# serizard/DeltaKD

Hardware: NVIDIA B200
Metric: distill-loss fwd+bwd samples/s (higher is better)
Workload: dtype bf16

## Files before the change

deltakd_b200/csrc/common.cuh:

```cuda
#pragma once
#include <cuda_bf16.h>
#include <cuda_runtime.h>
#include <stdint.h>
#include <stdio.h>

#include "../../include/deltakd.h"

#if defined(__CUDA_ARCH__) && (__CUDA_ARCH__ < 1000)
#error "libdeltakd_sm100 is written for sm_100a (B200) only"
#endif

namespace dkd {

void set_error(const char* fmt, ...);
int check_launch(const char* what);

#define DKD_REQUIRE(cond, code, ...)  \
  do {                                \
    if (!(cond)) {                    \
      ::dkd::set_error(__VA_ARGS__);  \
      return (code);                  \
    }                                 \
  } while (0)

// ... 164 lines not shown
__device__ __forceinline__ float2 add2(float2 a, float2 b) {
  unsigned long long r;
  asm("add.rn.f32x2 %0, %1, %2;" : "=l"(r) : "l"(f2_pack(a.x, a.y)), "l"(f2_pack(b.x, b.y)));
  return f2_unpack(r);
}
__device__ __forceinline__ float2 sub2(float2 a, float2 b) {
  unsigned long long r;
  asm("sub.rn.f32x2 %0, %1, %2;" : "=l"(r) : "l"(f2_pack(a.x, a.y)), "l"(f2_pack(b.x, b.y)));
  return f2_unpack(r);
}
__device__ __forceinline__ float2 mul2(float2 a, float2 b) {
  unsigned long long r;
  asm("mul.rn.f32x2 %0, %1, %2;" : "=l"(r) : "l"(f2_pack(a.x, a.y)), "l"(f2_pack(b.x, b.y)));
  return f2_unpack(r);
}
__device__ __forceinline__ float2 splat2(float x) { return make_float2(x, x); }

__device__ __forceinline__ float warp_sum(float v) {
#pragma unroll
  for (int o = 16; o > 0; o >>= 1) v += __shfl_xor_sync(0xffffffffu, v, o);
  return v;
}
__device__ __forceinline__ float warp_max(float v) {
#pragma unroll
  for (int o = 16; o > 0; o >>= 1) v = fmaxf(v, __shfl_xor_sync(0xffffffffu, v, o));
  return v;
}
__device__ __forceinline__ double warp_sum(double v) {
#pragma unroll
  for (int o = 16; o > 0; o >>= 1) v += __shfl_xor_sync(0xffffffffu, v, o);
  return v;
}

template <int K, int THREADS>
__device__ __forceinline__ void block_sum(float (&v)[K], float* scratch) {
  constexpr int WARPS = THREADS / 32;
  const int lane = threadIdx.x & 31, warp = threadIdx.x >> 5;
#pragma unroll
  for (int k = 0; k < K; ++k) v[k] = warp_sum(v[k]);
  if constexpr (THREADS == 32) return;
  __syncthreads();
  if (lane == 0) {
#pragma unroll
    for (int k = 0; k < K; ++k) scratch[k * WARPS + warp] = v[k];
  }
  __syncthreads();
#pragma unroll
  for (int k = 0; k < K; ++k) {
    float a = 0.f;
#pragma unroll
    for (int w = 0; w < WARPS; ++w) a += scratch[k * WARPS + w];
    v[k] = a;
  }
}
template <int K, int THREADS>
__device__ __forceinline__ void block_max(float (&v)[K], float* scratch) {
  constexpr int WARPS = THREADS / 32;
  const int lane = threadIdx.x & 31, warp = threadIdx.x >> 5;
#pragma unroll
  for (int k = 0; k < K; ++k) v[k] = warp_max(v[k]);
  if constexpr (THREADS == 32) return;
  __syncthreads();
  if (lane == 0) {
#pragma unroll
    for (int k = 0; k < K; ++k) scratch[k * WARPS + warp] = v[k];
  }
// ... 12 lines not shown
```

deltakd_b200/csrc/logit_kd.cu:

```cuda
#include <stdlib.h>

#include "common.cuh"

#ifndef DKD_LOGIT_STAMP
#define DKD_LOGIT_STAMP(point, dep) ((void)0)
#endif

namespace dkd {
namespace {

constexpr int kThreads = 128;

__device__ __forceinline__ float fexp(float x) {
  float y;
  asm("ex2.approx.ftz.f32 %0, %1;" : "=f"(y) : "f"(x * 1.4426950408889634f));
  return y;
}
__device__ __forceinline__ float fexp2(float x, float k2, float m2) {
  float y;
  asm("ex2.approx.ftz.f32 %0, %1;" : "=f"(y) : "f"(fmaf(x, k2, -m2)));
  return y;
}

__device__ __forceinline__ float2 ex2_2(float2 x) {
  float2 y;
  asm("ex2.approx.ftz.f32 %0, %1;" : "=f"(y.x) : "f"(x.x));
  asm("ex2.approx.ftz.f32 %0, %1;" : "=f"(y.y) : "f"(x.y));
  return y;
}

struct LogitKdParams {
  const void* z;
  const void* zk;
  const void* zt;
  const void* y;
  void* gz;
  void* gzk;
  float* loss_out;
  float* row_base;
  float* row_kd;
  unsigned int* ticket;
  int64_t B, C;
  int label_kind, kd_kind;
  float smoothing, alpha, tau;
  const float* mix_lam;
};

constexpr int kRuntimeMode = -2;
constexpr float kL2e = 1.4426950408889634f;
template <typename T, int VEC, int NV, int THREADS = kThreads, int LK = kRuntimeMode, int KK = kRuntimeMode,
          bool PACK2 = (THREADS == kThreads), typename Publish>
__device__ __forceinline__ void logit_row(const LogitKdParams& p, int64_t row, const T* z, const T* zk, const T* zt, const T* y,
                                          T* gz_row, T* gzk_row, float* scratch, int* s_arg, float* s_argv, float& base_out,
                                          float& kd_out, Publish&& publish) {
  const int64_t C = p.C;
  const int label_kind = LK == kRuntimeMode ? p.label_kind : LK;
  const int kd_kind = KK == kRuntimeMode ? p.kd_kind : KK;
  const int tid = THREADS == 32 ? (int)(threadIdx.x & 31) : (int)threadIdx.x;
  const int64_t label = label_kind == 1 ? reinterpret_cast<const int64_t*>(p.y)[row] : -1;
  const bool mixing = label_kind == 1 && p.mix_lam != nullptr;
  const int64_t label2 = mixing ? reinterpret_cast<const int64_t*>(p.y)[p.B - 1 - row] : -1;
  const float lam = mixing ? __ldg(p.mix_lam) : 1.f;
  const float invT = kd_kind == 1 ? 1.f / p.tau : 1.f;

  constexpr int NVR = NV > 0 ? NV : 1;
  float rz[NVR][VEC], rk[NVR][VEC], rt[NVR][VEC], ry[NVR][VEC];
  const int nchunk = (int)((C + (int64_t)THREADS * VEC - 1) / ((int64_t)THREADS * VEC));

  auto col_of = [&](int it) -> int64_t { return ((int64_t)it * THREADS + tid) * VEC; };
  const T* any = label_kind >= 0 ? z : zk;
  const T* lz = label_kind >= 0 ? z : any;
  const T* lzk = kd_kind ? zk : any;
  const T* lzt = kd_kind ? zt : any;
  const T* ly = label_kind == 0 ? y : any;
  auto load4 = [&](int it, float (&a)[VEC], float (&b)[VEC], float (&c)[VEC], float (&d)[VEC]) {
    const int64_t col0 = col_of(it);
    const int64_t col = col0 < C ? col0 : 0;
    Vec<T, VEC>::load(lz + col, a);
    Vec<T, VEC>::load(lzk + col, b);
    Vec<T, VEC>::load(lzt + col, c);
    Vec<T, VEC>::load(ly + col, d);
    if (label_kind < 0) {
#pragma unroll
      for (int v = 0; v < VEC; ++v) a[v] = 0.f;
    }
  };

  float mx[3] = {-INFINITY, -INFINITY, -INFINITY};
  float best = -INFINITY;
  int64_t best_i = INT64_MAX;
  auto pass1 = [&](int it, float (&a)[VEC], float (&b)[VEC], float (&c)[VEC]) {
    const int64_t col = col_of(it);
    if (col < C) {
#pragma unroll
      for (int v = 0; v < VEC; ++v) {
        mx[0] = fmaxf(mx[0], a[v]);
        if (kd_kind) {
          mx[1] = fmaxf(mx[1], b[v]);
          mx[2] = fmaxf(mx[2], c[v]);
          if (kd_kind == 2 && c[v] > best) { best = c[v]; best_i = col + v; }
        }
      }
    }
  };
  if constexpr (NV > 0) {
#pragma unroll
    for (int it = 0; it < NV; ++it)
      if (it < nchunk) load4(it, rz[it], rk[it], rt[it], ry[it]);
#pragma unroll
    for (int it = 0; it < NV; ++it)
      if (it < nchunk) pass1(it, rz[it], rk[it], rt[it]);
  } else {
    for (int it = 0; it < nchunk; ++it) {
      load4(it, rz[0], rk[0], rt[0], ry[0]);
      pass1(it, rz[0], rk[0], rt[0]);
    }
  }
  DKD_LOGIT_STAMP(1, mx[0]);
  block_max<3, THREADS>(mx, scratch);
  DKD_LOGIT_STAMP(2, mx[0]);
  mx[1] *= invT;
  mx[2] *= invT;
  int64_t tgt = label;
  int64_t hard_idx = -1;
  if (kd_kind == 2) {
    float bv = best;
    long long bi = (long long)best_i;
#pragma unroll
    for (int o = 16; o > 0; o >>= 1) {
      float ov = __shfl_xor_sync(0xffffffffu, bv, o);
      long long oi = __shfl_xor_sync(0xffffffffu, bi, o);
      if (ov > bv || (ov == bv && oi < bi)) { bv = ov; bi = oi; }
    }
    if constexpr (THREADS > 32) {
      __syncthreads();
      if ((threadIdx.x & 31) == 0) { s_argv[threadIdx.x >> 5] = bv; s_arg[threadIdx.x >> 5] = (int)bi; }
      __syncthreads();
      bv = s_argv[0]; bi = s_arg[0];
#pragma unroll
      for (int w = 1; w < THREADS / 32; ++w) {
        if (s_argv[w] > bv || (s_argv[w] == bv && s_arg[w] < bi)) { bv = s_argv[w]; bi = s_arg[w]; }
      }
    }
    hard_idx = bi;
  }
  (void)tgt;

  float st8[8] = {0.f, 0.f, 0.f, 0.f, 0.f, 0.f, 0.f, 0.f};
  float (&s)[4] = *reinterpret_cast<float(*)[4]>(&st8[0]);
  float (&t)[4] = *reinterpret_cast<float(*)[4]>(&st8[4]);
  constexpr bool PACKED = NV > 0 && VEC % 2 == 0 && PACK2;
  float2 S2[4], T2[2];
#pragma unroll
  for (int k = 0; k < 4; ++k) S2[k] = make_float2(0.f, 0.f);
  T2[0] = T2[1] = make_float2(0.f, 0.f);
  auto pass2 = [&](int it, float (&a)[VEC], float (&b)[VEC], float (&c)[VEC], float (&d)[VEC]) {
    const int64_t col = col_of(it);
    if (col < C) {
      if constexpr (PACKED) {
        const float2 kz = splat2(kL2e), nm0 = splat2(-mx[0] * kL2e);
        const float2 kt = splat2(invT * kL2e), nm1 = splat2(-mx[1] * kL2e), nm2 = splat2(-mx[2] * kL2e);
#pragma unroll
        for (int v = 0; v < VEC; v += 2) {
          const float2 A = make_float2(a[v], a[v + 1]);
          const float2 ea = ex2_2(fma2(A, kz, nm0));
          S2[0] = add2(S2[0], ea);
          if (label_kind == 0) {
            const float2 D = make_float2(d[v], d[v + 1]);
            T2[0] = add2(T2[0], D);
            T2[1] = fma2(D, A, T2[1]);
          } else {
            T2[1] = add2(T2[1], A);
            if (col + v == label) t[2] = a[v];
            if (col + v + 1 == label) t[2] = a[v + 1];
            if (col + v == label2) t[0] = a[v];
            if (col + v + 1 == label2) t[0] = a[v + 1];
          }
          a[v] = ea.x; a[v + 1] = ea.y;
          if (kd_kind == 1) {
            const float2 Bv = make_float2(b[v], b[v + 1]), Cv = make_float2(c[v], c[v + 1]);
            const float2 eb = ex2_2(fma2(Cv, kt, nm2)), es = ex2_2(fma2(Bv, kt, nm1));
            S2[1] = add2(S2[1], es);
            S2[2] = add2(S2[2], eb);
            S2[3] = fma2(eb, sub2(Cv, Bv), S2[3]);
            b[v] = es.x; b[v + 1] = es.y;
            c[v] = eb.x; c[v + 1] = eb.y;
          } else if (kd_kind == 2) {
            const float2 Bv = make_float2(b[v], b[v + 1]);
            const float2 es = ex2_2(fma2(Bv, kz, nm1));
            S2[1] = add2(S2[1], es);
            if (col + v == hard_idx) t[3] = b[v];
            if (col + v + 1 == hard_idx) t[3] = b[v + 1];
            b[v] = es.x; b[v + 1] = es.y;
          }
        }
        return;
      }
#pragma unroll
      for (int v = 0; v < VEC; ++v) {
        const float ea = fexp2(a[v], kL2e, mx[0] * kL2e);
        s[0] += ea;
        if (label_kind == 0) { t[0] += d[v]; t[1] += d[v] * a[v]; }
        else { t[1] += a[v]; if (col + v == label) t[2] = a[v]; if (col + v == label2) t[0] = a[v]; }
        if (NV > 0) a[v] = ea;
        if (kd_kind == 1) {
          const float eb = fexp2(c[v], invT * kL2e, mx[2] * kL2e), es = fexp2(b[v], invT * kL2e, mx[1] * kL2e);
          s[1] += es;
          s[2] += eb;
          s[3] = fmaf(eb, c[v] - b[v], s[3]);
          if (NV > 0) { b[v] = es; c[v] = eb; }
        } else if (kd_kind == 2) {
          const float es = fexp2(b[v], kL2e, mx[1] * kL2e);
          s[1] += es;
          if (col + v == hard_idx) t[3] = b[v];
          if (NV > 0) b[v] = es;
        }
      }
    }
  };
  if constexpr (NV > 0) {
#pragma unroll
    for (int it = 0; it < NV; ++it) if (it < nchunk) pass2(it, rz[it], rk[it], rt[it], ry[it]);
  } else {
    for (int it = 0; it < nchunk; ++it) {
      load4(it, rz[0], rk[0], rt[0], ry[0]);
      pass2(it, rz[0], rk[0], rt[0], ry[0]);
    }
  }
  if constexpr (PACKED) {
#pragma unroll
    for (int k = 0; k < 4; ++k) s[k] = S2[k].x + S2[k].y;
    if (label_kind == 0) t[0] = T2[0].x + T2[0].y;
    t[1] = T2[1].x + T2[1].y;
  }
  block_sum<8, THREADS>(st8, scratch);
  DKD_LOGIT_STAMP(3, s[0]);
  s[3] *= invT;

  const float Bf = (float)p.B, Cf = (float)C;
  const float lse0 = mx[0] + __logf(s[0]);
  float base_row, kd_row = 0.f;
  if (label_kind < 0) base_row = 0.f;
  else if (label_kind == 0) base_row = lse0 * t[0] - t[1];
  else base_row = (1.f - p.smoothing) * (lse0 - (lam * t[2] + (1.f - lam) * t[0])) + p.smoothing * (lse0 - t[1] / Cf);
  float lse1 = 0.f, lse2 = 0.f;
  if (kd_kind == 1) {
    lse1 = mx[1] + __logf(s[1]);
    lse2 = mx[2] + __logf(s[2]);
    kd_row = __fdividef(s[3], s[2]) - lse2 + lse1;
  } else if (kd_kind == 2) {
    lse1 = mx[1] + __logf(s[1]);
    kd_row = lse1 - t[3];
  }
  publish(base_row, kd_row);

  const float wb = (kd_kind == 0 ? 1.f : 1.f - p.alpha) / Bf;
  const float wk = kd_kind == 1 ? p.alpha * p.tau / (Bf * Cf) : p.alpha / Bf;
  const float inv_s0 = __frcp_rn(s[0]), inv_s1 = kd_kind ? __frcp_rn(s[1]) : 0.f, inv_s2 = kd_kind == 1 ? __frcp_rn(s[2]) : 0.f;
  const float k0 = (label_kind == 0 ? inv_s0 * t[0] : inv_s0) * wb;
  const float k1 = inv_s1 * wk, k2 = inv_s2 * wk;
  const float sm_wb = p.smoothing / Cf * wb, hot_wb = (1.f - p.smoothing) * wb * lam, hot2_wb = (1.f - p.smoothing) * wb * (1.f - lam);
  T* gz = label_kind >= 0 ? gz_row : nullptr;
  T* gzk = kd_kind ? gzk_row : nullptr;
  auto pass3 = [&](int it, float (&a)[VEC], float (&b)[VEC], float (&c)[VEC], float (&d)[VEC]) {
    const int64_t col = col_of(it);
    if (col < C) {
      float g0[VEC], g1[VEC];
      if constexpr (PACKED) {
        const float2 K0 = splat2(k0), K1 = splat2(k1), NK2 = splat2(-k2), NWB = splat2(-wb), NSM = splat2(-sm_wb);
#pragma unroll
        for (int v = 0; v < VEC; v += 2) {
          const float2 e0 = make_float2(a[v], a[v + 1]);
          float2 r0;
          if (label_kind == 0) r0 = fma2(e0, K0, mul2(make_float2(d[v], d[v + 1]), NWB));
          else {
            r0 = fma2(e0, K0, NSM);
            if (col + v == label) r0.x -= hot_wb;
            if (col + v + 1 == label) r0.y -= hot_wb;
            if (col + v == label2) r0.x -= hot2_wb;
            if (col + v + 1 == label2) r0.y -= hot2_wb;
          }
          g0[v] = r0.x; g0[v + 1] = r0.y;
          if (kd_kind == 1) {
            const float2 r1 = fma2(make_float2(b[v], b[v + 1]), K1, mul2(make_float2(c[v], c[v + 1]), NK2));
            g1[v] = r1.x; g1[v + 1] = r1.y;
          } else if (kd_kind == 2) {
            float2 r1 = mul2(make_float2(b[v], b[v + 1]), K1);
            if (col + v == hard_idx) r1.x -= wk;
            if (col + v + 1 == hard_idx) r1.y -= wk;
            g1[v] = r1.x; g1[v + 1] = r1.y;
          }
        }
      } else {
// ... 3 lines not shown
        if (label_kind == 0) g0[v] = fmaf(e0, k0, -(d[v] * wb));
        else g0[v] = fmaf(e0, k0, -sm_wb) - (col + v == label ? hot_wb : 0.f) - (col + v == label2 ? hot2_wb : 0.f);
        if (kd_kind == 1) {
          const float es = NV > 0 ? b[v] : fexp(b[v] * invT - mx[1]);
          const float et = NV > 0 ? c[v] : fexp(c[v] * invT - mx[2]);
          g1[v] = fmaf(es, k1, -(et * k2));
        } else if (kd_kind == 2) {
          const float es = NV > 0 ? b[v] : fexp(b[v] - mx[1]);
          g1[v] = fmaf(es, k1, col + v == hard_idx ? -wk : 0.f);
        }
      }
      }
      if (gz) Vec<T, VEC>::store(gz + col, g0);
      if (gzk) Vec<T, VEC>::store(gzk + col, g1);
    }
  };
  if (gz || gzk) {
    if constexpr (NV > 0) {
#pragma unroll
      for (int it = 0; it < NV; ++it) if (it < nchunk) pass3(it, rz[it], rk[it], rt[it], ry[it]);
    } else {
      for (int it = 0; it < nchunk; ++it) {
        load4(it, rz[0], rk[0], rt[0], ry[0]);
        pass3(it, rz[0], rk[0], rt[0], ry[0]);
      }
    }
  }
  DKD_LOGIT_STAMP(4, 0.f);

  base_out = base_row;
  kd_out = kd_row;
}

__device__ __forceinline__ unsigned int take_ticket(unsigned int* ticket) {
  unsigned int old;
  asm volatile("atom.acq_rel.gpu.global.add.u32 %0, [%1], 1;" : "=r"(old) : "l"(ticket) : "memory");
  return old;
}

template <int THREADS = kThreads>
__device__ __forceinline__ void logit_fold(const LogitKdParams& p, float* scratch, int64_t n_part) {
  const float Bf = (float)p.B, Cf = (float)p.C;
  float acc[2] = {0.f, 0.f};
  auto batch = [&](int64_t r0) {
    float b[8], k[8];
#pragma unroll
    for (int u = 0; u < 8; ++u) {
      const int64_t r = r0 + (int64_t)u * THREADS;
      b[u] = r < n_part ? __ldcg(p.row_base + r) : 0.f;
      k[u] = r < n_part ? __ldcg(p.row_kd + r) : 0.f;
    }
#pragma unroll
    for (int u = 0; u < 8; ++u) { acc[0] += b[u]; acc[1] += k[u]; }
  };
  batch(threadIdx.x);
  for (int64_t r0 = threadIdx.x + 8 * THREADS; r0 < n_part; r0 += 8 * THREADS) batch(r0);
  DKD_LOGIT_STAMP(6, acc[0]);
  block_sum<2, THREADS>(acc, scratch);
  if (threadIdx.x == 0) {
    const float base = acc[0] / Bf;
    float kd = 0.f, total = base;
    if (p.kd_kind == 1) { kd = acc[1] * p.tau * p.tau / (Bf * Cf); total = base * (1.f - p.alpha) + kd * p.alpha; }
    else if (p.kd_kind == 2) { kd = acc[1] / Bf; total = base * (1.f - p.alpha) + kd * p.alpha; }
    p.loss_out[0] = total;
    p.loss_out[1] = base;
    p.loss_out[2] = kd;
    *p.ticket = 0u;
    DKD_LOGIT_STAMP(7, 0.f);
  }
}

template <int THREADS>
__device__ __forceinline__ void logit_finalize(const LogitKdParams& p, float* scratch, bool* s_last, int64_t n_part) {
  if (threadIdx.x == 0) {
    __threadfence();
    const unsigned int done = atomicAdd(p.ticket, 1u);
    *s_last = (done == gridDim.x - 1);
  }
  __syncthreads();
  if (!*s_last) return;
  __threadfence();
  logit_fold<THREADS>(p, scratch, n_part);
}

__device__ __forceinline__ void logit_finalize_any(const LogitKdParams& p, float* scratch, bool* s_last, int64_t n_part) {
  const float Bf = (float)p.B, Cf = (float)p.C;
  if (threadIdx.x == 0) {
    __threadfence();
    const unsigned int done = atomicAdd(p.ticket, 1u);
    *s_last = (done == gridDim.x - 1);
  }
  __syncthreads();
  if (!*s_last || threadIdx.x >= 32) return;
  __threadfence();
  float a0 = 0.f, a1 = 0.f;
  for (int64_t r = threadIdx.x; r < n_part; r += 32) { a0 += __ldcg(p.row_base + r); a1 += __ldcg(p.row_kd + r); }
  a0 = warp_sum(a0); a1 = warp_sum(a1);
  if (threadIdx.x == 0) {
    const float base = a0 / Bf;
    float kd = 0.f, total = base;
    if (p.kd_kind == 1) { kd = a1 * p.tau * p.tau / (Bf * Cf); total = base * (1.f - p.alpha) + kd * p.alpha; }
    else if (p.kd_kind == 2) { kd = a1 / Bf; total = base * (1.f - p.alpha) + kd * p.alpha; }
    p.loss_out[0] = total; p.loss_out[1] = base; p.loss_out[2] = kd;
    *p.ticket = 0u;
  }
}

constexpr int kFoldThreads = 1024;
__global__ void __launch_bounds__(kFoldThreads) logit_fold_kernel(LogitKdParams p) {
  __shared__ float scratch[2 * (kFoldThreads / 32)];
  float a0[8], a1[8];
#pragma unroll
  for (int u = 0; u < 8; ++u) a0[u] = a1[u] = 0.f;
  for (int64_t r0 = threadIdx.x; r0 < p.B; r0 += 8 * kFoldThreads) {
#pragma unroll
    for (int u = 0; u < 8; ++u) {
      const int64_t r = r0 + (int64_t)u * kFoldThreads;
      if (r < p.B) { a0[u] += __ldcg(p.row_base + r); a1[u] += __ldcg(p.row_kd + r); }
    }
  }
  float acc[2] = {((a0[0] + a0[1]) + (a0[2] + a0[3])) + ((a0[4] + a0[5]) + (a0[6] + a0[7])),
                  ((a1[0] + a1[1]) + (a1[2] + a1[3])) + ((a1[4] + a1[5]) + (a1[6] + a1[7]))};
  block_sum<2, kFoldThreads>(acc, scratch);
  if (threadIdx.x == 0) {
    const float Bf = (float)p.B, Cf = (float)p.C;
    const float base = acc[0] / Bf;
    float kd = 0.f, total = base;
    if (p.kd_kind == 1) { kd = acc[1] * p.tau * p.tau / (Bf * Cf); total = base * (1.f - p.alpha) + kd * p.alpha; }
    else if (p.kd_kind == 2) { kd = acc[1] / Bf; total = base * (1.f - p.alpha) + kd * p.alpha; }
    p.loss_out[0] = total;
    p.loss_out[1] = base;
    p.loss_out[2] = kd;
  }
}

template <typename T, int VEC, int NV, int THREADS = kThreads, bool TICKET = true, int LK = kRuntimeMode, int KK = kRuntimeMode>
__global__ void __launch_bounds__(THREADS) logit_kd_kernel(LogitKdParams p) {
  __shared__ float scratch[8 * (kThreads / 32)];
  __shared__ int s_arg[kThreads / 32];
  __shared__ float s_argv[kThreads / 32];
  __shared__ bool s_last;
  DKD_LOGIT_STAMP(0, 0.f);
  grid_dep_wait();
  DKD_LOGIT_STAMP(8, 0.f);
  grid_dep_launch();
  const int64_t row = blockIdx.x, C = p.C;
  const T* z = p.label_kind >= 0 ? reinterpret_cast<const T*>(p.z) + row * C : nullptr;
  const T* zk = p.kd_kind ? reinterpret_cast<const T*>(p.zk) + row * C : nullptr;
  const T* zt = p.kd_kind ? reinterpret_cast<const T*>(p.zt) + row * C : nullptr;
  const T* y = p.label_kind == 0 ? reinterpret_cast<const T*>(p.y) + row * C : nullptr;
  T* gz = p.gz ? reinterpret_cast<T*>(p.gz) + row * C : nullptr;
  T* gzk = p.gzk ? reinterpret_cast<T*>(p.gzk) + row * C : nullptr;
  float base_row, kd_row;
  unsigned int done = 0;
  logit_row<T, VEC, NV, THREADS, LK, KK>(p, row, z, zk, zt, y, gz, gzk, scratch, s_arg, s_argv, base_row, kd_row,
                                         [&](float base, float kd) {
                                           if (threadIdx.x == 0) {
                                             p.row_base[row] = base;
                                             p.row_kd[row] = kd;
                                             if (TICKET) done = take_ticket(p.ticket);
                                           }
                                         });
  if (TICKET) {
    if (threadIdx.x == 0) {
      DKD_LOGIT_STAMP(5, (float)done);
      s_last = (done == gridDim.x - 1);
    }
    __syncthreads();
    if (s_last) logit_fold<THREADS>(p, scratch, p.B);
  }
}

constexpr int kRingStages = 3;
constexpr int kRingMaxWarps = 8;
constexpr int kRingSmemBudget = 224 * 1024;

__device__ __forceinline__ void bulk_g2s(void* dst, const void* src, uint32_t bytes, uint64_t* bar) {
  asm volatile("cp.async.bulk.shared::cluster.global.mbarrier::complete_tx::bytes [%0], [%1], %2, [%3];" ::"r"(
                   (uint32_t)__cvta_generic_to_shared(dst)),
               "l"(src), "r"(bytes), "r"((uint32_t)__cvta_generic_to_shared(bar))
               : "memory");
}
__device__ __forceinline__ void bulk_s2g(void* dst, const void* src, uint32_t bytes) {
  asm volatile("cp.async.bulk.global.shared::cta.bulk_group [%0], [%1], %2;" ::"l"(dst), "r"((uint32_t)__cvta_generic_to_shared(src)),
               "r"(bytes)
               : "memory");
}
__device__ __forceinline__ void ring_bar_init(uint64_t* bar) {
  asm volatile("mbarrier.init.shared::cta.b64 [%0], 1;" ::"r"((uint32_t)__cvta_generic_to_shared(bar)) : "memory");
}
__device__ __forceinline__ void ring_bar_expect(uint64_t* bar, uint32_t bytes) {
  asm volatile("mbarrier.arrive.expect_tx.shared::cta.b64 _, [%0], %1;" ::"r"((uint32_t)__cvta_generic_to_shared(bar)), "r"(bytes) : "memory");
}
__device__ __forceinline__ void ring_bar_wait(uint64_t* bar, uint32_t parity) {
  const uint32_t a = (uint32_t)__cvta_generic_to_shared(bar);
  uint32_t ok = 0;
  const long long t0 = clock64();
  while (true) {
    asm volatile(
        "{\n\t.reg .pred p;\n\t"
        "mbarrier.try_wait.parity.shared::cta.b64 p, [%1], %2;\n\t"
        "selp.u32 %0, 1, 0, p;\n\t}"
        : "=r"(ok)
// ... 59 lines not shown
    float base_row, kd_row;
    logit_row<T, VEC, NV, 32, LK, KK, true>(p, row, LK >= 0 ? sz : nullptr, KK ? szk : nullptr, KK ? szt : nullptr, LK == 0 ? sy : nullptr,
                                            (p.gz && LK >= 0) ? sz : nullptr, (p.gzk && KK) ? szk : nullptr, nullptr, nullptr, nullptr,
                                            base_row, kd_row, [](float, float) {});
    acc_base += base_row;
    acc_kd += kd_row;
    asm volatile("fence.proxy.async.shared::cta;" ::: "memory");
    __syncwarp();
    if (lane == 0) {
      const int64_t off = row * C;
      if (p.gz && LK >= 0) bulk_s2g(reinterpret_cast<T*>(p.gz) + off, sz, row_bytes);
      if (p.gzk && KK) bulk_s2g(reinterpret_cast<T*>(p.gzk) + off, szk, row_bytes);
      asm volatile("cp.async.bulk.commit_group;" ::: "memory");
      asm volatile("cp.async.bulk.wait_group.read 1;" ::: "memory");
      if (k + kRingStages - 1 < nrows) issue(k + kRingStages - 1);
    }
    __syncwarp();
  }
  if (lane == 0) {
    asm volatile("cp.async.bulk.wait_group 0;" ::: "memory");
    if (gw < p.B) {
      p.row_base[gw] = acc_base;
      p.row_kd[gw] = acc_kd;
    }
  }
  const int64_t n_part = GW < p.B ? GW : p.B;
  __shared__ float scratch[2 * kRingMaxWarps];
  __shared__ bool s_last;
  __syncthreads();
  if (blockDim.x == 32 * kRingMaxWarps) logit_finalize<32 * kRingMaxWarps>(p, scratch, &s_last, n_part);
  else logit_finalize_any(p, scratch, &s_last, n_part);
}

template <typename T, int VEC, int THREADS, bool TICKET, int LK, int KK>
void launch_nv(const LogitKdParams& p, int64_t nchunk, dim3 grid, cudaStream_t stream) {
  if (nchunk <= 1) launch_pdl(logit_kd_kernel<T, VEC, 1, THREADS, TICKET, LK, KK>, grid, dim3(THREADS), stream, p);
  else if (nchunk <= 2) launch_pdl(logit_kd_kernel<T, VEC, 2, THREADS, TICKET, LK, KK>, grid, dim3(THREADS), stream, p);
  else launch_pdl(logit_kd_kernel<T, VEC, 4, THREADS, TICKET, LK, KK>, grid, dim3(THREADS), stream, p);
}
template <typename T, int VEC, int THREADS, bool TICKET>
void launch_mode(const LogitKdParams& p, int64_t nchunk, dim3 grid, cudaStream_t stream) {
  if constexpr (VEC * sizeof(T) == 16) {
    const int lk = p.label_kind, kk = p.kd_kind;
    if (lk == 0 && kk == 1) return launch_nv<T, VEC, THREADS, TICKET, 0, 1>(p, nchunk, grid, stream);
    if (lk == 1 && kk == 1) return launch_nv<T, VEC, THREADS, TICKET, 1, 1>(p, nchunk, grid, stream);
    if (lk == 0 && kk == 2) return launch_nv<T, VEC, THREADS, TICKET, 0, 2>(p, nchunk, grid, stream);
    if (lk == 1 && kk == 2) return launch_nv<T, VEC, THREADS, TICKET, 1, 2>(p, nchunk, grid, stream);
    if (lk == 0 && kk == 0) return launch_nv<T, VEC, THREADS, TICKET, 0, 0>(p, nchunk, grid, stream);
    if (lk == 1 && kk == 0) return launch_nv<T, VEC, THREADS, TICKET, 1, 0>(p, nchunk, grid, stream);
  }
  launch_nv<T, VEC, THREADS, TICKET, kRuntimeMode, kRuntimeMode>(p, nchunk, grid, stream);
}

template <typename T, int VEC, int NV, int LK, int KK>
int launch_ring_mode(const LogitKdParams& p, cudaStream_t stream) {
  constexpr int NOPS = (LK >= 0 ? 1 : 0) + (LK == 0 ? 1 : 0) + (KK ? 2 : 0);
  const int row_stride = (int)((p.C * (int64_t)sizeof(T) + 127) / 128 * 128);
  int warps = kRingSmemBudget / (kRingStages * NOPS * row_stride);
  if (warps > kRingMaxWarps) warps = kRingMaxWarps;
  if (warps < 2) return 1;
  const size_t smem = (size_t)warps * kRingStages * NOPS * row_stride + (size_t)warps * kRingStages * sizeof(uint64_t);
  int64_t grid = (p.B + warps - 1) / warps;
  if (grid > kNumSMs) grid = kNumSMs;
  auto kern = logit_ring_kernel<T, VEC, NV, LK, KK>;
  cudaFuncSetAttribute(kern, cudaFuncAttributeMaxDynamicSharedMemorySize, (int)smem);
  kern<<<(unsigned)grid, 32 * warps, smem, stream>>>(p, row_stride);
  return 0;
}
template <typename T, int VEC, int NV>
int launch_ring(const LogitKdParams& p, cudaStream_t stream) {
  const int lk = p.label_kind, kk = p.kd_kind;
  if (lk == 0 && kk == 1) return launch_ring_mode<T, VEC, NV, 0, 1>(p, stream);
  if (lk == 1 && kk == 1) return launch_ring_mode<T, VEC, NV, 1, 1>(p, stream);
  if (lk == 0 && kk == 2) return launch_ring_mode<T, VEC, NV, 0, 2>(p, stream);
  if (lk == 1 && kk == 2) return launch_ring_mode<T, VEC, NV, 1, 2>(p, stream);
  if (lk == 0 && kk == 0) return launch_ring_mode<T, VEC, NV, 0, 0>(p, stream);
  if (lk == 1 && kk == 0) return launch_ring_mode<T, VEC, NV, 1, 0>(p, stream);
  return 1;
}
bool ring_enabled() {
  static const bool on = [] { const char* e = getenv("DKD_LOGIT_RING"); return !(e && e[0] == '0'); }();
  return on;
}

template <typename T, int VEC>
int launch_logit_kd(const LogitKdParams& p, cudaStream_t stream) {
  const int64_t per_chunk = (int64_t)kThreads * VEC;
  const int64_t nchunk = (p.C + per_chunk - 1) / per_chunk;
  dim3 grid((unsigned)p.B), block(kThreads);
  const int64_t nchunk64 = (p.C + 64 * VEC - 1) / (64 * VEC);
  if constexpr (VEC * sizeof(T) == 16) {
    constexpr int NV = 32 / VEC;
    if (p.B >= 1024 && p.C * (int64_t)sizeof(T) >= 1024 && p.C <= 32 * VEC * NV && ring_enabled()) {
      if (launch_ring<T, VEC, NV>(p, stream) == 0) return check_launch("dkd_logit_kd_fwdbwd: ring");
    }
  }
  if (p.B >= 1024 && nchunk64 <= 4) {
    launch_mode<T, VEC, 64, false>(p, nchunk64, grid, stream);
    int rc = check_launch("dkd_logit_kd_fwdbwd");
    if (rc != DKD_OK) return rc;
    logit_fold_kernel<<<1, kFoldThreads, 0, stream>>>(p);
    return check_launch("dkd_logit_kd_fwdbwd: fold");
  }
  if (nchunk <= 4) launch_mode<T, VEC, kThreads, true>(p, nchunk, grid, stream);
  else launch_pdl(logit_kd_kernel<T, VEC, 0>, grid, block, stream, p);
  return check_launch("dkd_logit_kd_fwdbwd");
}

template <typename T>
int dispatch_vec(const LogitKdParams& p, cudaStream_t stream) {
  constexpr int MAXV = 16 / (int)sizeof(T);
  auto aligned = [&](int vec) {
    const uintptr_t m = (uintptr_t)vec * sizeof(T) - 1;
    auto ok = [&](const void* q) { return q == nullptr || (((uintptr_t)q) & m) == 0; };
    return p.C % vec == 0 && ok(p.z) && ok(p.zk) && ok(p.zt) && (p.label_kind == 1 || ok(p.y)) && ok(p.gz) && ok(p.gzk);
  };
  if (aligned(MAXV)) return launch_logit_kd<T, MAXV>(p, stream);
  if (aligned(MAXV / 2)) return launch_logit_kd<T, MAXV / 2>(p, stream);
  return launch_logit_kd<T, 1>(p, stream);
}

}
}

extern "C" {

size_t dkd_logit_kd_workspace_bytes(int64_t B) {
  return (size_t)(B > 0 ? B : 0) * 2 * sizeof(float) + 256;
}

int dkd_logit_kd_fwdbwd(const void* outputs, const void* outputs_kd, const void* teacher_logits,
                        const void* labels, int label_kind, int kd_kind, int64_t B, int64_t C, int dtype,
                        float smoothing, float alpha, float tau, const float* mix_lam, void* g_outputs, void* g_outputs_kd,
                        float* loss_out, void* workspace, size_t workspace_bytes, dkd_stream_t stream) {
  using namespace dkd;
  int rc = dkd_check_device();
  if (rc != DKD_OK) return rc;
  DKD_REQUIRE(B > 0 && C > 0 && B < (1ll << 31), DKD_E_SHAPE, "dkd_logit_kd_fwdbwd: bad shape B=%lld C=%lld", (long long)B, (long long)C);
  DKD_REQUIRE(dtype == DKD_F32 || dtype == DKD_BF16, DKD_E_DTYPE, "dkd_logit_kd_fwdbwd: dtype %d", dtype);
// ... 24 lines not shown
```

Measured before the change: 42.97 million.

## Merge row max and sum reductions with online rescale and offload ticket to tail warp

For multi-warp rows, the separate block max barrier is removed. Each warp now computes local maxima and rescaled partial sums, and a single named-barrier exchange merges them with exp rescaling. The gradient scale factors absorb the difference between the local and row maxima. The argmax is folded into the same exchange, carrying the hard-label logit with it. An extra tail warp per block waits on a named barrier, writes the row partials, takes the ticket and does a warp-only fold. This takes the atomic and the final fold off the compute warps' critical path, at the cost of more threads per block and approximate rescale math.

```diff
diff --git a/deltakd_b200/csrc/common.cuh b/deltakd_b200/csrc/common.cuh
--- a/deltakd_b200/csrc/common.cuh
+++ b/deltakd_b200/csrc/common.cuh
@@ -220,6 +220,9 @@
   return v;
 }
 
+__device__ __forceinline__ void bar_sync(int id, int n) { asm volatile("bar.sync %0, %1;" ::"r"(id), "r"(n) : "memory"); }
+__device__ __forceinline__ void bar_arrive(int id, int n) { asm volatile("bar.arrive %0, %1;" ::"r"(id), "r"(n) : "memory"); }
+
 template <int K, int THREADS>
 __device__ __forceinline__ void block_sum(float (&v)[K], float* scratch) {
   constexpr int WARPS = THREADS / 32;
diff --git a/deltakd_b200/csrc/logit_kd.cu b/deltakd_b200/csrc/logit_kd.cu
--- a/deltakd_b200/csrc/logit_kd.cu
+++ b/deltakd_b200/csrc/logit_kd.cu
@@ -10,6 +10,8 @@
 namespace {
 
 constexpr int kThreads = 128;
+constexpr int kRowBar = 1;
+constexpr int kTailBar = 2;
 
 __device__ __forceinline__ float fexp(float x) {
   float y;
@@ -27,6 +29,12 @@
   asm("ex2.approx.ftz.f32 %0, %1;" : "=f"(y.x) : "f"(x.x));
   asm("ex2.approx.ftz.f32 %0, %1;" : "=f"(y.y) : "f"(x.y));
   return y;
+}
+
+__device__ __forceinline__ float rescale(float m, float M) {
+  float y;
+  asm("ex2.approx.ftz.f32 %0, %1;" : "=f"(y) : "f"((m - M) * 1.4426950408889634f));
+  return m == -INFINITY ? 0.f : y;
 }
 
 struct LogitKdParams {
@@ -87,7 +95,7 @@
   };
 
   float mx[3] = {-INFINITY, -INFINITY, -INFINITY};
-  float best = -INFINITY;
+  float best = -INFINITY, best_k = 0.f;
   int64_t best_i = INT64_MAX;
   auto pass1 = [&](int it, float (&a)[VEC], float (&b)[VEC], float (&c)[VEC]) {
     const int64_t col = col_of(it);
@@ -98,7 +106,11 @@
         if (kd_kind) {
           mx[1] = fmaxf(mx[1], b[v]);
           mx[2] = fmaxf(mx[2], c[v]);
-          if (kd_kind == 2 && c[v] > best) { best = c[v]; best_i = col + v; }
+          if (kd_kind == 2 && c[v] > best) {
+            best = c[v];
+            best_i = col + v;
+            if constexpr (THREADS > 32) best_k = b[v];
+          }
         }
       }
     }
@@ -117,30 +129,24 @@
     }
   }
   DKD_LOGIT_STAMP(1, mx[0]);
-  block_max<3, THREADS>(mx, scratch);
-  DKD_LOGIT_STAMP(2, mx[0]);
+  if constexpr (THREADS == 32) {
+    block_max<3, THREADS>(mx, scratch);
+    DKD_LOGIT_STAMP(2, mx[0]);
+  }
   mx[1] *= invT;
   mx[2] *= invT;
   int64_t tgt = label;
   int64_t hard_idx = -1;
+  float bv = best, bk = best_k;
+  long long bi = (long long)best_i;
   if (kd_kind == 2) {
-    float bv = best;
-    long long bi = (long long)best_i;
 #pragma unroll
     for (int o = 16; o > 0; o >>= 1) {
       float ov = __shfl_xor_sync(0xffffffffu, bv, o);
       long long oi = __shfl_xor_sync(0xffffffffu, bi, o);
-      if (ov > bv || (ov == bv && oi < bi)) { bv = ov; bi = oi; }
-    }
-    if constexpr (THREADS > 32) {
-      __syncthreads();
-      if ((threadIdx.x & 31) == 0) { s_argv[threadIdx.x >> 5] = bv; s_arg[threadIdx.x >> 5] = (int)bi; }
-      __syncthreads();
-      bv = s_argv[0]; bi = s_arg[0];
-#pragma unroll
-      for (int w = 1; w < THREADS / 32; ++w) {
-        if (s_argv[w] > bv || (s_argv[w] == bv && s_arg[w] < bi)) { bv = s_argv[w]; bi = s_arg[w]; }
-      }
+      float ok = 0.f;
+      if constexpr (THREADS > 32) ok = __shfl_xor_sync(0xffffffffu, bk, o);
+      if (ov > bv || (ov == bv && oi < bi)) { bv = ov; bi = oi; bk = ok; }
     }
     hard_idx = bi;
   }
@@ -189,8 +195,8 @@
             const float2 Bv = make_float2(b[v], b[v + 1]);
             const float2 es = ex2_2(fma2(Bv, kz, nm1));
             S2[1] = add2(S2[1], es);
-            if (col + v == hard_idx) t[3] = b[v];
-            if (col + v + 1 == hard_idx) t[3] = b[v + 1];
+            if (THREADS == 32 && col + v == hard_idx) t[3] = b[v];
+            if (THREADS == 32 && col + v + 1 == hard_idx) t[3] = b[v + 1];
             b[v] = es.x; b[v + 1] = es.y;
           }
         }
@@ -212,7 +218,7 @@
         } else if (kd_kind == 2) {
           const float es = fexp2(b[v], kL2e, mx[1] * kL2e);
           s[1] += es;
-          if (col + v == hard_idx) t[3] = b[v];
+          if (THREADS == 32 && col + v == hard_idx) t[3] = b[v];
           if (NV > 0) b[v] = es;
         }
       }
@@ -233,7 +239,67 @@
     if (label_kind == 0) t[0] = T2[0].x + T2[0].y;
     t[1] = T2[1].x + T2[1].y;
   }
-  block_sum<8, THREADS>(st8, scratch);
+  float fr[3] = {1.f, 1.f, 1.f};
+  if constexpr (THREADS == 32) {
+    block_sum<8, THREADS>(st8, scratch);
+  } else {
+    constexpr int WARPS = THREADS / 32, NS = 3 + 8;
+    const int lane = threadIdx.x & 31, warp = threadIdx.x >> 5;
+    float mw[3];
+#pragma unroll
+    for (int k = 0; k < 3; ++k) {
+      mw[k] = warp_max(mx[k]);
+      const float f = rescale(mx[k], mw[k]);
+      s[k] *= f;
+      if (k == 2) s[3] *= f;
+    }
+#pragma unroll
+    for (int k = 0; k < 8; ++k) st8[k] = warp_sum(st8[k]);
+    if (lane == 0) {
+      float* w = scratch + warp * NS;
+#pragma unroll
+      for (int k = 0; k < 3; ++k) w[k] = mw[k];
+#pragma unroll
+      for (int k = 0; k < 8; ++k) w[3 + k] = st8[k];
+      if (kd_kind == 2) { s_argv[warp] = bv; s_arg[warp] = (int)bi; w[3 + 7] = bk; }
+    }
+    bar_sync(kRowBar, THREADS);
+    float M[3] = {-INFINITY, -INFINITY, -INFINITY};
+#pragma unroll
+    for (int w = 0; w < WARPS; ++w) {
+#pragma unroll
+      for (int k = 0; k < 3; ++k) M[k] = fmaxf(M[k], scratch[w * NS + k]);
+    }
+#pragma unroll
+    for (int k = 0; k < 8; ++k) st8[k] = 0.f;
+#pragma unroll
+    for (int w = 0; w < WARPS; ++w) {
+      const float* ws = scratch + w * NS;
+      const float f0 = rescale(ws[0], M[0]), f1 = rescale(ws[1], M[1]), f2 = rescale(ws[2], M[2]);
+      s[0] += ws[3] * f0;
+      s[1] += ws[4] * f1;
+      s[2] += ws[5] * f2;
+      s[3] += ws[6] * f2;
+#pragma unroll
+      for (int k = 4; k < 8; ++k) st8[k] += ws[3 + k];
+    }
+    if (kd_kind == 2) {
+      int wb = 0;
+      bv = s_argv[0]; bi = s_arg[0];
+#pragma unroll
+      for (int w = 1; w < WARPS; ++w) {
+        if (s_argv[w] > bv || (s_argv[w] == bv && s_arg[w] < bi)) { bv = s_argv[w]; bi = s_arg[w]; wb = w; }
+      }
+      hard_idx = bi;
+      t[3] = scratch[wb * NS + 3 + 7];
+    }
+    if constexpr (NV > 0) {
+#pragma unroll
+      for (int k = 0; k < 3; ++k) fr[k] = rescale(mx[k], M[k]);
+    }
+#pragma unroll
+    for (int k = 0; k < 3; ++k) mx[k] = M[k];
+  }
   DKD_LOGIT_STAMP(3, s[0]);
   s[3] *= invT;
 
@@ -257,8 +323,8 @@
   const float wb = (kd_kind == 0 ? 1.f : 1.f - p.alpha) / Bf;
   const float wk = kd_kind == 1 ? p.alpha * p.tau / (Bf * Cf) : p.alpha / Bf;
   const float inv_s0 = __frcp_rn(s[0]), inv_s1 = kd_kind ? __frcp_rn(s[1]) : 0.f, inv_s2 = kd_kind == 1 ? __frcp_rn(s[2]) : 0.f;
-  const float k0 = (label_kind == 0 ? inv_s0 * t[0] : inv_s0) * wb;
-  const float k1 = inv_s1 * wk, k2 = inv_s2 * wk;
+  const float k0 = (label_kind == 0 ? inv_s0 * t[0] : inv_s0) * wb * fr[0];
+  const float k1 = inv_s1 * wk * fr[1], k2 = inv_s2 * wk * fr[2];
   const float sm_wb = p.smoothing / Cf * wb, hot_wb = (1.f - p.smoothing) * wb * lam, hot2_wb = (1.f - p.smoothing) * wb * (1.f - lam);
   T* gz = label_kind >= 0 ? gz_row : nullptr;
   T* gzk = kd_kind ? gzk_row : nullptr;
@@ -334,9 +400,19 @@
   return old;
 }
 
+__device__ __forceinline__ void store_loss(const LogitKdParams& p, float sum_base, float sum_kd) {
+  const float Bf = (float)p.B, Cf = (float)p.C;
+  const float base = sum_base / Bf;
+  float kd = 0.f, total = base;
+  if (p.kd_kind == 1) { kd = sum_kd * p.tau * p.tau / (Bf * Cf); total = base * (1.f - p.alpha) + kd * p.alpha; }
+  else if (p.kd_kind == 2) { kd = sum_kd / Bf; total = base * (1.f - p.alpha) + kd * p.alpha; }
+  p.loss_out[0] = total;
+  p.loss_out[1] = base;
+  p.loss_out[2] = kd;
+}
+
 template <int THREADS = kThreads>
 __device__ __forceinline__ void logit_fold(const LogitKdParams& p, float* scratch, int64_t n_part) {
-  const float Bf = (float)p.B, Cf = (float)p.C;
   float acc[2] = {0.f, 0.f};
   auto batch = [&](int64_t r0) {
     float b[8], k[8];
@@ -351,16 +427,44 @@
   };
   batch(threadIdx.x);
   for (int64_t r0 = threadIdx.x + 8 * THREADS; r0 < n_part; r0 += 8 * THREADS) batch(r0);
-  DKD_LOGIT_STAMP(6, acc[0]);
   block_sum<2, THREADS>(acc, scratch);
   if (threadIdx.x == 0) {
-    const float base = acc[0] / Bf;
-    float kd = 0.f, total = base;
-    if (p.kd_kind == 1) { kd = acc[1] * p.tau * p.tau / (Bf * Cf); total = base * (1.f - p.alpha) + kd * p.alpha; }
-    else if (p.kd_kind == 2) { kd = acc[1] / Bf; total = base * (1.f - p.alpha) + kd * p.alpha; }
-    p.loss_out[0] = total;
-    p.loss_out[1] = base;
-    p.loss_out[2] = kd;
+    store_loss(p, acc[0], acc[1]);
+    *p.ticket = 0u;
+  }
+}
+
+template <int VT>
+__device__ __forceinline__ void logit_fold_warp(const LogitKdParams& p, int64_t n_part) {
+  constexpr int NW = VT / 32;
+  const int lane = threadIdx.x & 31;
+  float acc[NW][2];
+#pragma unroll
+  for (int j = 0; j < NW; ++j) acc[j][0] = acc[j][1] = 0.f;
+  for (int64_t r0 = 0; r0 < n_part; r0 += 8 * VT) {
+    float b[NW][8], k[NW][8];
+#pragma unroll
+    for (int u = 0; u < 8; ++u) {
+      const bool any = r0 + (int64_t)u * VT < n_part;
+#pragma unroll
+      for (int j = 0; j < NW; ++j) {
+        const int64_t r = r0 + lane + 32 * j + (int64_t)u * VT;
+        b[j][u] = any && r < n_part ? __ldcg(p.row_base + r) : 0.f;
+        k[j][u] = any && r < n_part ? __ldcg(p.row_kd + r) : 0.f;
+      }
+    }
+#pragma unroll
+    for (int j = 0; j < NW; ++j) {
+#pragma unroll
+      for (int u = 0; u < 8; ++u) { acc[j][0] += b[j][u]; acc[j][1] += k[j][u]; }
+    }
+  }
+  DKD_LOGIT_STAMP(6, acc[0][0]);
+  float sum[2] = {0.f, 0.f};
+#pragma unroll
+  for (int j = 0; j < NW; ++j) { sum[0] += warp_sum(acc[j][0]); sum[1] += warp_sum(acc[j][1]); }
+  if (lane == 0) {
+    store_loss(p, sum[0], sum[1]);
     *p.ticket = 0u;
     DKD_LOGIT_STAMP(7, 0.f);
   }
@@ -430,17 +534,33 @@
   }
 }
 
+constexpr int logit_block(int threads, bool ticket) { return threads + (ticket ? 32 : 0); }
+
 template <typename T, int VEC, int NV, int THREADS = kThreads, bool TICKET = true, int LK = kRuntimeMode, int KK = kRuntimeMode>
-__global__ void __launch_bounds__(THREADS) logit_kd_kernel(LogitKdParams p) {
-  __shared__ float scratch[8 * (kThreads / 32)];
+__global__ void __launch_bounds__(logit_block(THREADS, TICKET)) logit_kd_kernel(LogitKdParams p) {
+  __shared__ float scratch[(3 + 8) * (kThreads / 32)];
   __shared__ int s_arg[kThreads / 32];
   __shared__ float s_argv[kThreads / 32];
-  __shared__ bool s_last;
+  __shared__ float s_part[2];
   DKD_LOGIT_STAMP(0, 0.f);
   grid_dep_wait();
   DKD_LOGIT_STAMP(8, 0.f);
   grid_dep_launch();
   const int64_t row = blockIdx.x, C = p.C;
+  if (TICKET && threadIdx.x >= THREADS) {
+    bar_sync(kTailBar, logit_block(THREADS, TICKET));
+    DKD_LOGIT_STAMP(9, s_part[0]);
+    unsigned int done = 0;
+    if (threadIdx.x == THREADS) {
+      p.row_base[row] = s_part[0];
+      p.row_kd[row] = s_part[1];
+      done = take_ticket(p.ticket);
+      DKD_LOGIT_STAMP(5, (float)done);
+    }
+    __syncwarp();
+    if (__shfl_sync(0xffffffffu, done, 0) == gridDim.x - 1) logit_fold_warp<THREADS>(p, p.B);
+    return;
+  }
   const T* z = p.label_kind >= 0 ? reinterpret_cast<const T*>(p.z) + row * C : nullptr;
   const T* zk = p.kd_kind ? reinterpret_cast<const T*>(p.zk) + row * C : nullptr;
   const T* zt = p.kd_kind ? reinterpret_cast<const T*>(p.zt) + row * C : nullptr;
@@ -448,23 +568,16 @@
   T* gz = p.gz ? reinterpret_cast<T*>(p.gz) + row * C : nullptr;
   T* gzk = p.gzk ? reinterpret_cast<T*>(p.gzk) + row * C : nullptr;
   float base_row, kd_row;
-  unsigned int done = 0;
   logit_row<T, VEC, NV, THREADS, LK, KK>(p, row, z, zk, zt, y, gz, gzk, scratch, s_arg, s_argv, base_row, kd_row,
                                          [&](float base, float kd) {
-                                           if (threadIdx.x == 0) {
+                                           if (TICKET) {
+                                             if (threadIdx.x == 0) { s_part[0] = base; s_part[1] = kd; }
+                                             bar_arrive(kTailBar, logit_block(THREADS, TICKET));
+                                           } else if (threadIdx.x == 0) {
                                              p.row_base[row] = base;
                                              p.row_kd[row] = kd;
-                                             if (TICKET) done = take_ticket(p.ticket);
                                            }
                                          });
-  if (TICKET) {
-    if (threadIdx.x == 0) {
-      DKD_LOGIT_STAMP(5, (float)done);
-      s_last = (done == gridDim.x - 1);
-    }
-    __syncthreads();
-    if (s_last) logit_fold<THREADS>(p, scratch, p.B);
-  }
 }
 
 constexpr int kRingStages = 3;
@@ -592,9 +705,10 @@
 
 template <typename T, int VEC, int THREADS, bool TICKET, int LK, int KK>
 void launch_nv(const LogitKdParams& p, int64_t nchunk, dim3 grid, cudaStream_t stream) {
-  if (nchunk <= 1) launch_pdl(logit_kd_kernel<T, VEC, 1, THREADS, TICKET, LK, KK>, grid, dim3(THREADS), stream, p);
-  else if (nchunk <= 2) launch_pdl(logit_kd_kernel<T, VEC, 2, THREADS, TICKET, LK, KK>, grid, dim3(THREADS), stream, p);
-  else launch_pdl(logit_kd_kernel<T, VEC, 4, THREADS, TICKET, LK, KK>, grid, dim3(THREADS), stream, p);
+  const dim3 block(logit_block(THREADS, TICKET));
+  if (nchunk <= 1) launch_pdl(logit_kd_kernel<T, VEC, 1, THREADS, TICKET, LK, KK>, grid, block, stream, p);
+  else if (nchunk <= 2) launch_pdl(logit_kd_kernel<T, VEC, 2, THREADS, TICKET, LK, KK>, grid, block, stream, p);
+  else launch_pdl(logit_kd_kernel<T, VEC, 4, THREADS, TICKET, LK, KK>, grid, block, stream, p);
 }
 template <typename T, int VEC, int THREADS, bool TICKET>
 void launch_mode(const LogitKdParams& p, int64_t nchunk, dim3 grid, cudaStream_t stream) {
@@ -645,7 +759,7 @@
 int launch_logit_kd(const LogitKdParams& p, cudaStream_t stream) {
   const int64_t per_chunk = (int64_t)kThreads * VEC;
   const int64_t nchunk = (p.C + per_chunk - 1) / per_chunk;
-  dim3 grid((unsigned)p.B), block(kThreads);
+  dim3 grid((unsigned)p.B), block(logit_block(kThreads, true));
   const int64_t nchunk64 = (p.C + 64 * VEC - 1) / (64 * VEC);
   if constexpr (VEC * sizeof(T) == 16) {
     constexpr int NV = 32 / VEC;
```

New measurement: 41.37 million, median of 6. 0.963x the previous value.

## Replace atomic ticket fold with PDL fold kernel and add L2 prefetch of rows

Applied to the files above, without the earlier changes.

Removes the last-block atomic ticket reduction from the per-row logit KD kernel and runs the final loss reduction in a separate single-block fold kernel launched with programmatic dependent launch. The large-B path's fold kernel now also uses PDL. Each row block issues an L2 bulk prefetch for its input rows before the grid dependency wait, so loads overlap the previous kernel's tail. Removing the atomic drops per-block serialization, but the small-B path gains an extra kernel launch.

```diff
diff --git a/deltakd_b200/csrc/logit_kd.cu b/deltakd_b200/csrc/logit_kd.cu
--- a/deltakd_b200/csrc/logit_kd.cu
+++ b/deltakd_b200/csrc/logit_kd.cu
@@ -4,6 +4,9 @@
 
 #ifndef DKD_LOGIT_STAMP
 #define DKD_LOGIT_STAMP(point, dep) ((void)0)
+#endif
+#ifndef DKD_LOGIT_FOLD_STAMP
+#define DKD_LOGIT_FOLD_STAMP(point, dep) ((void)0)
 #endif
 
 namespace dkd {
@@ -328,12 +331,6 @@
   kd_out = kd_row;
 }
 
-__device__ __forceinline__ unsigned int take_ticket(unsigned int* ticket) {
-  unsigned int old;
-  asm volatile("atom.acq_rel.gpu.global.add.u32 %0, [%1], 1;" : "=r"(old) : "l"(ticket) : "memory");
-  return old;
-}
-
 template <int THREADS = kThreads>
 __device__ __forceinline__ void logit_fold(const LogitKdParams& p, float* scratch, int64_t n_part) {
   const float Bf = (float)p.B, Cf = (float)p.C;
@@ -351,7 +348,7 @@
   };
   batch(threadIdx.x);
   for (int64_t r0 = threadIdx.x + 8 * THREADS; r0 < n_part; r0 += 8 * THREADS) batch(r0);
-  DKD_LOGIT_STAMP(6, acc[0]);
+  DKD_LOGIT_FOLD_STAMP(6, acc[0]);
   block_sum<2, THREADS>(acc, scratch);
   if (threadIdx.x == 0) {
     const float base = acc[0] / Bf;
@@ -361,8 +358,7 @@
     p.loss_out[0] = total;
     p.loss_out[1] = base;
     p.loss_out[2] = kd;
-    *p.ticket = 0u;
-    DKD_LOGIT_STAMP(7, 0.f);
+    DKD_LOGIT_FOLD_STAMP(7, 0.f);
   }
 }
 
@@ -377,6 +373,7 @@
   if (!*s_last) return;
   __threadfence();
   logit_fold<THREADS>(p, scratch, n_part);
+  if (threadIdx.x == 0) *p.ticket = 0u;
 }
 
 __device__ __forceinline__ void logit_finalize_any(const LogitKdParams& p, float* scratch, bool* s_last, int64_t n_part) {
@@ -402,9 +399,19 @@
   }
 }
 
+__global__ void __launch_bounds__(kThreads) logit_fold_small_kernel(LogitKdParams p) {
+  __shared__ float scratch[2 * (kThreads / 32)];
+  grid_dep_wait();
+  DKD_LOGIT_FOLD_STAMP(9, 0.f);
+  grid_dep_launch();
+  logit_fold<kThreads>(p, scratch, p.B);
+}
+
 constexpr int kFoldThreads = 1024;
 __global__ void __launch_bounds__(kFoldThreads) logit_fold_kernel(LogitKdParams p) {
   __shared__ float scratch[2 * (kFoldThreads / 32)];
+  grid_dep_wait();
+  grid_dep_launch();
   float a0[8], a1[8];
 #pragma unroll
   for (int u = 0; u < 8; ++u) a0[u] = a1[u] = 0.f;
@@ -430,41 +437,48 @@
   }
 }
 
-template <typename T, int VEC, int NV, int THREADS = kThreads, bool TICKET = true, int LK = kRuntimeMode, int KK = kRuntimeMode>
+template <int THREADS>
+__device__ __forceinline__ void prefetch_l2(const void* src, int64_t bytes) {
+  const uintptr_t a = reinterpret_cast<uintptr_t>(src);
+  if (((a | (uintptr_t)bytes) & 15) == 0) {
+    const uint32_t n = (uint32_t)min(bytes, (int64_t)0xfffffff0);
+    if (threadIdx.x == 0) asm volatile("cp.async.bulk.prefetch.L2.global [%0], %1;" ::"l"(src), "r"(n) : "memory");
+  } else {
+    for (uintptr_t l = (a & ~(uintptr_t)127) + (uintptr_t)threadIdx.x * 128; l < a + (uintptr_t)bytes; l += THREADS * 128)
+      asm volatile("prefetch.global.L2 [%0];" ::"l"(l));
+  }
+}
+
+template <typename T, int VEC, int NV, int THREADS = kThreads, int LK = kRuntimeMode, int KK = kRuntimeMode>
 __global__ void __launch_bounds__(THREADS) logit_kd_kernel(LogitKdParams p) {
   __shared__ float scratch[8 * (kThreads / 32)];
   __shared__ int s_arg[kThreads / 32];
   __shared__ float s_argv[kThreads / 32];
-  __shared__ bool s_last;
   DKD_LOGIT_STAMP(0, 0.f);
+  const int label_kind = LK == kRuntimeMode ? p.label_kind : LK;
+  const int kd_kind = KK == kRuntimeMode ? p.kd_kind : KK;
+  const int64_t row = blockIdx.x, C = p.C;
+  const T* z = label_kind >= 0 ? reinterpret_cast<const T*>(p.z) + row * C : nullptr;
+  const T* zk = kd_kind ? reinterpret_cast<const T*>(p.zk) + row * C : nullptr;
+  const T* zt = kd_kind ? reinterpret_cast<const T*>(p.zt) + row * C : nullptr;
+  const T* y = label_kind == 0 ? reinterpret_cast<const T*>(p.y) + row * C : nullptr;
+  T* gz = p.gz ? reinterpret_cast<T*>(p.gz) + row * C : nullptr;
+  T* gzk = p.gzk ? reinterpret_cast<T*>(p.gzk) + row * C : nullptr;
+  const T* rows[4] = {z, zk, zt, y};
+#pragma unroll
+  for (int i = 0; i < 4; ++i)
+    if (rows[i]) prefetch_l2<THREADS>(rows[i], C * (int64_t)sizeof(T));
   grid_dep_wait();
   DKD_LOGIT_STAMP(8, 0.f);
   grid_dep_launch();
-  const int64_t row = blockIdx.x, C = p.C;
-  const T* z = p.label_kind >= 0 ? reinterpret_cast<const T*>(p.z) + row * C : nullptr;
-  const T* zk = p.kd_kind ? reinterpret_cast<const T*>(p.zk) + row * C : nullptr;
-  const T* zt = p.kd_kind ? reinterpret_cast<const T*>(p.zt) + row * C : nullptr;
-  const T* y = p.label_kind == 0 ? reinterpret_cast<const T*>(p.y) + row * C : nullptr;
-  T* gz = p.gz ? reinterpret_cast<T*>(p.gz) + row * C : nullptr;
-  T* gzk = p.gzk ? reinterpret_cast<T*>(p.gzk) + row * C : nullptr;
   float base_row, kd_row;
-  unsigned int done = 0;
   logit_row<T, VEC, NV, THREADS, LK, KK>(p, row, z, zk, zt, y, gz, gzk, scratch, s_arg, s_argv, base_row, kd_row,
                                          [&](float base, float kd) {
                                            if (threadIdx.x == 0) {
                                              p.row_base[row] = base;
                                              p.row_kd[row] = kd;
-                                             if (TICKET) done = take_ticket(p.ticket);
                                            }
                                          });
-  if (TICKET) {
-    if (threadIdx.x == 0) {
-      DKD_LOGIT_STAMP(5, (float)done);
-      s_last = (done == gridDim.x - 1);
-    }
-    __syncthreads();
-    if (s_last) logit_fold<THREADS>(p, scratch, p.B);
-  }
 }
 
 constexpr int kRingStages = 3;
@@ -590,24 +604,24 @@
   else logit_finalize_any(p, scratch, &s_last, n_part);
 }
 
-template <typename T, int VEC, int THREADS, bool TICKET, int LK, int KK>
+template <typename T, int VEC, int THREADS, int LK, int KK>
 void launch_nv(const LogitKdParams& p, int64_t nchunk, dim3 grid, cudaStream_t stream) {
-  if (nchunk <= 1) launch_pdl(logit_kd_kernel<T, VEC, 1, THREADS, TICKET, LK, KK>, grid, dim3(THREADS), stream, p);
-  else if (nchunk <= 2) launch_pdl(logit_kd_kernel<T, VEC, 2, THREADS, TICKET, LK, KK>, grid, dim3(THREADS), stream, p);
-  else launch_pdl(logit_kd_kernel<T, VEC, 4, THREADS, TICKET, LK, KK>, grid, dim3(THREADS), stream, p);
-}
-template <typename T, int VEC, int THREADS, bool TICKET>
+  if (nchunk <= 1) launch_pdl(logit_kd_kernel<T, VEC, 1, THREADS, LK, KK>, grid, dim3(THREADS), stream, p);
+  else if (nchunk <= 2) launch_pdl(logit_kd_kernel<T, VEC, 2, THREADS, LK, KK>, grid, dim3(THREADS), stream, p);
+  else launch_pdl(logit_kd_kernel<T, VEC, 4, THREADS, LK, KK>, grid, dim3(THREADS), stream, p);
+}
+template <typename T, int VEC, int THREADS>
 void launch_mode(const LogitKdParams& p, int64_t nchunk, dim3 grid, cudaStream_t stream) {
   if constexpr (VEC * sizeof(T) == 16) {
     const int lk = p.label_kind, kk = p.kd_kind;
-    if (lk == 0 && kk == 1) return launch_nv<T, VEC, THREADS, TICKET, 0, 1>(p, nchunk, grid, stream);
-    if (lk == 1 && kk == 1) return launch_nv<T, VEC, THREADS, TICKET, 1, 1>(p, nchunk, grid, stream);
-    if (lk == 0 && kk == 2) return launch_nv<T, VEC, THREADS, TICKET, 0, 2>(p, nchunk, grid, stream);
-    if (lk == 1 && kk == 2) return launch_nv<T, VEC, THREADS, TICKET, 1, 2>(p, nchunk, grid, stream);
-    if (lk == 0 && kk == 0) return launch_nv<T, VEC, THREADS, TICKET, 0, 0>(p, nchunk, grid, stream);
-    if (lk == 1 && kk == 0) return launch_nv<T, VEC, THREADS, TICKET, 1, 0>(p, nchunk, grid, stream);
-  }
-  launch_nv<T, VEC, THREADS, TICKET, kRuntimeMode, kRuntimeMode>(p, nchunk, grid, stream);
+    if (lk == 0 && kk == 1) return launch_nv<T, VEC, THREADS, 0, 1>(p, nchunk, grid, stream);
+    if (lk == 1 && kk == 1) return launch_nv<T, VEC, THREADS, 1, 1>(p, nchunk, grid, stream);
+    if (lk == 0 && kk == 2) return launch_nv<T, VEC, THREADS, 0, 2>(p, nchunk, grid, stream);
+    if (lk == 1 && kk == 2) return launch_nv<T, VEC, THREADS, 1, 2>(p, nchunk, grid, stream);
+    if (lk == 0 && kk == 0) return launch_nv<T, VEC, THREADS, 0, 0>(p, nchunk, grid, stream);
+    if (lk == 1 && kk == 0) return launch_nv<T, VEC, THREADS, 1, 0>(p, nchunk, grid, stream);
+  }
+  launch_nv<T, VEC, THREADS, kRuntimeMode, kRuntimeMode>(p, nchunk, grid, stream);
 }
 
 template <typename T, int VEC, int NV, int LK, int KK>
@@ -654,15 +668,18 @@
     }
   }
   if (p.B >= 1024 && nchunk64 <= 4) {
-    launch_mode<T, VEC, 64, false>(p, nchunk64, grid, stream);
+    launch_mode<T, VEC, 64>(p, nchunk64, grid, stream);
     int rc = check_launch("dkd_logit_kd_fwdbwd");
     if (rc != DKD_OK) return rc;
-    logit_fold_kernel<<<1, kFoldThreads, 0, stream>>>(p);
+    launch_pdl(logit_fold_kernel, dim3(1), dim3(kFoldThreads), stream, p);
     return check_launch("dkd_logit_kd_fwdbwd: fold");
   }
-  if (nchunk <= 4) launch_mode<T, VEC, kThreads, true>(p, nchunk, grid, stream);
+  if (nchunk <= 4) launch_mode<T, VEC, kThreads>(p, nchunk, grid, stream);
   else launch_pdl(logit_kd_kernel<T, VEC, 0>, grid, block, stream, p);
-  return check_launch("dkd_logit_kd_fwdbwd");
+  int rc = check_launch("dkd_logit_kd_fwdbwd");
+  if (rc != DKD_OK) return rc;
+  launch_pdl(logit_fold_small_kernel, dim3(1), dim3(kThreads), stream, p);
+  return check_launch("dkd_logit_kd_fwdbwd: fold");
 }
 
 template <typename T>
```

Result: faster. 44.38 million before, 48.47 million after, median of 6 (+9.2%).
